# fernandezdaniel/MOBOCMF

Hardware: AMD Instinct MI355X
Metric: ELBO steps/sec (MFDGP d=8 M=512 N=8192 S=8) (higher is better)
Workload: dtype f64

## Files before the change

### include/mobocmf_hip.h

```cpp
#ifndef MOBOCMF_HIP_H
#define MOBOCMF_HIP_H

#include <stddef.h>
#include <stdint.h>

#ifdef __cplusplus
extern "C" {
#endif

typedef void* mobocmf_stream_t;

#define MOBOCMF_MAX_D 32
#define MOBOCMF_MAX_XDIV 48

enum {
    MOBOCMF_OK = 0,
    MOBOCMF_BAD_ARG = 1,
    MOBOCMF_WORKSPACE_TOO_SMALL = 2,
    MOBOCMF_HIP_ERROR = 3,
    MOBOCMF_NOT_PD = 4,
    MOBOCMF_BAD_ARCH = 5
};

typedef struct mobocmf_tuning {
    uint32_t struct_size;
    int32_t small_gemm_max;
    int32_t small_panel_max;
    int32_t tile_rows;
    int32_t pair_mode;
    int32_t mid_gemm_max;
    int32_t mid_gemm_waves;
    int32_t syrk_workgroups;
    int32_t sparse_backward;
    int32_t potrf_cols;
} mobocmf_tuning;
int mobocmf_tuning_init(mobocmf_tuning* t);

typedef struct {
    int32_t kind;
    int32_t d;
    int32_t M;
    int32_t xdiv;
    int64_t Np;
    int32_t branch;
    int32_t want_dx;
    double jitter;
    double min_var;
    int32_t phase;
    int32_t reserved;
    const mobocmf_tuning* tuning;
    void* const* probe_events;
} mobocmf_layer_desc;
#define MOBOCMF_PROBE_EVENTS 11

#define MOBOCMF_PHASE_ALL 0
#define MOBOCMF_PHASE_CHAIN 1
#define MOBOCMF_PHASE_PANEL 2
#define MOBOCMF_PHASE_CHAIN_ONLY 3
#define MOBOCMF_PHASE_PANEL_INPUTS 4

int mobocmf_version(void);
int mobocmf_device_arch_ok(void);

int mobocmf_layer_workspace_bytes(const mobocmf_layer_desc* desc, size_t* saved_bytes, size_t* scratch_bytes);

int mobocmf_layer_chain_state_bytes(const mobocmf_layer_desc* desc, size_t* bytes);

// ... 381 lines not shown
```

### mobocmf_amd/_lib.py

```python
import ctypes
import os

_HERE = os.path.dirname(os.path.abspath(__file__))
LIB_PATH = os.environ.get("MOBOCMF_HIP_LIB") or os.path.join(_HERE, "csrc", "libmobocmf_hip.so")

OK, BAD_ARG, WORKSPACE_TOO_SMALL, HIP_ERROR, NOT_PD, BAD_ARCH = range(6)
_ERR = {1: "MOBOCMF_BAD_ARG", 2: "MOBOCMF_WORKSPACE_TOO_SMALL", 3: "MOBOCMF_HIP_ERROR", 4: "MOBOCMF_NOT_PD",
        5: "MOBOCMF_BAD_ARCH"}


class Tuning(ctypes.Structure):
    _fields_ = [("struct_size", ctypes.c_uint32), ("small_gemm_max", ctypes.c_int32), ("small_panel_max", ctypes.c_int32),
                ("tile_rows", ctypes.c_int32), ("pair_mode", ctypes.c_int32), ("mid_gemm_max", ctypes.c_int32),
                ("mid_gemm_waves", ctypes.c_int32), ("syrk_workgroups", ctypes.c_int32), ("sparse_backward", ctypes.c_int32),
                ("potrf_cols", ctypes.c_int32)]
    KNOBS = tuple(n for n, _ in _fields_[1:])

    def copy(self):
        t = Tuning()
        ctypes.memmove(ctypes.byref(t), ctypes.byref(self), ctypes.sizeof(Tuning))
        return t


PROBE_EVENTS = 11


class LayerDesc(ctypes.Structure):
    _fields_ = [("kind", ctypes.c_int32), ("d", ctypes.c_int32), ("M", ctypes.c_int32), ("xdiv", ctypes.c_int32),
                ("Np", ctypes.c_int64), ("branch", ctypes.c_int32), ("want_dx", ctypes.c_int32),
                ("jitter", ctypes.c_double), ("min_var", ctypes.c_double), ("phase", ctypes.c_int32),
                ("reserved", ctypes.c_int32), ("tuning", ctypes.POINTER(Tuning)), ("probe_events", ctypes.c_void_p)]


TINY_MAX_LAYERS, TINY_MAX_M, TINY_MAX_D = 3, 32, 8
COOP_MAX_M = 128
FROZEN_MAX_M = 512
FROZEN_SPLIT_MAX_M = 1024
STEP_GRADIENTS, STEP_UPDATE, STEP_FORWARD, STEP_INPUT_GRADIENTS, STEP_COUPLED = range(5)
STEP_CHAIN_VALID = 16


class TinyModel(ctypes.Structure):
    _L = TINY_MAX_LAYERS
    _fields_ = [("L", ctypes.c_int32), ("M", ctypes.c_int32), ("d", ctypes.c_int32), ("S", ctypes.c_int32),
                ("N", ctypes.c_int32), ("rows", ctypes.c_int32 * _L), ("trainable", ctypes.c_uint32 * _L),
                ("branch", ctypes.c_int32),
                ("x", ctypes.c_void_p), ("y", ctypes.c_void_p), ("fid", ctypes.c_void_p), ("Zx", ctypes.c_void_p),
                ("raw", (ctypes.c_void_p * 7) * _L), ("m", ctypes.c_void_p * _L), ("L_S", ctypes.c_void_p * _L),
                ("raw_noise", ctypes.c_void_p * _L), ("noise_lo", ctypes.c_double * _L), ("noise_hi", ctypes.c_double * _L),
# ... 215 lines not shown
```

### mobocmf_amd/csrc/api.hip

```cpp
#include "common.h"

static const mobocmf_tuning kDefaultTuning = {(uint32_t)sizeof(mobocmf_tuning), 384, 512, 0, 0, 1024, 32, 0, 1, 0};
static thread_local const mobocmf_tuning* t_tuning = nullptr;
static thread_local void* const* t_probe = nullptr;
const mobocmf_tuning& tune() { return t_tuning ? *t_tuning : kDefaultTuning; }
bool tuning_ok(const mobocmf_tuning* t) {
    if (!t) return true;
    return t->struct_size == sizeof(mobocmf_tuning) && t->small_gemm_max >= 1 && t->small_gemm_max <= 512 &&
           t->small_panel_max >= 1 && t->small_panel_max <= 512 && (t->tile_rows == 0 || t->tile_rows == 64 || t->tile_rows == 128) &&
           t->pair_mode >= 0 && t->pair_mode <= 2 && t->mid_gemm_max >= 0 && t->mid_gemm_max <= 4096 &&
           (t->mid_gemm_waves == 4 || t->mid_gemm_waves == 8 || t->mid_gemm_waves == 32) &&
           (t->syrk_workgroups == 0 || (t->syrk_workgroups >= 16 && t->syrk_workgroups <= 4096)) &&
           (t->sparse_backward == 0 || t->sparse_backward == 1) && (t->potrf_cols == 0 || t->potrf_cols == 1 || t->potrf_cols == 4);
}
TuneScope::TuneScope(const mobocmf_tuning* t, void* const* probe) : prev_t(t_tuning), prev_p(t_probe) {
    t_tuning = t;
    t_probe = probe;
}
TuneScope::~TuneScope() {
    t_tuning = prev_t;
    t_probe = prev_p;
}
void probe_at(int i, hipStream_t s) {
    if (t_probe && i < MOBOCMF_PROBE_EVENTS && t_probe[i]) (void)hipEventRecord((hipEvent_t)t_probe[i], s);
}
static void set_pairing(GemmArgs& g) { g.pair_mode = tune().pair_mode; }
static int panel_tile_rows(int, int64_t) { return tune().tile_rows; }

#define TRY(x)              \
    do {                    \
        int _rc = (x);      \
        if (_rc) return _rc; \
    } while (0)

namespace {

struct Bump {
    uintptr_t base;
    size_t off, cap;
    bool ok;
    Bump(void* p, size_t c) : base((uintptr_t)p), off(0), cap(c), ok(true) {}
    double* take(int64_t n) {
        size_t bytes = ((size_t)n * sizeof(double) + 255) & ~(size_t)255;
        if (bytes > cap || off > cap - bytes) { ok = false; off += bytes; return nullptr; }
        double* r = base ? (double*)(base + off) : nullptr;
        off += bytes;
        return r;
    }
};

struct Dims {
    int M, Mp, nrb, H;
    int64_t N, Np, nbase;
    int splitk;
    dim3 ggrid_mn, ggrid_mm;
};

GemmArgs gemm_args(const double* A, int64_t lda, const double* B, int64_t ldb, double* C, int64_t ldc, int Mr, int64_t Nc,
                   int64_t Kd, int tri, double alpha) {
    GemmArgs g = {};
    g.A = A; g.lda = lda; g.B = B; g.ldb = ldb; g.C = C; g.ldc = ldc;
    g.Mr = Mr; g.Nc = Nc; g.Kd = Kd; g.tri = tri; g.alpha = alpha;
    return g;
}

int syrk_splitk(int Mp, int64_t Np, int* sD) {
    const int nrb = Mp / TILE;
    const int64_t nF = (int64_t)nrb * (nrb - 1) / 2, nD = nrb, ksteps = Np / 16;
    int cap = (int)(ksteps / 8);
    if (cap > 128) cap = 128;
    if (cap < 1) cap = 1;
    *sD = 0;
    if (nF == 0) {
        int sk = 512 < cap ? 512 : cap;
        if (sk >= 8) sk &= ~7;
        return sk;
    }
    int budget = tune().syrk_workgroups;
    if (budget <= 0) budget = Np <= 16384 ? 256 : 512;
    double best = 1e30;
    int bF = 1, bD = 1;
    for (int f = 1; f <= cap; ++f)
        for (int d = 1; d <= f; ++d) {
            if (nF * f + nD * d > budget) break;
            const double cf = (double)((ksteps + f - 1) / f), cd = 0.625 * (double)((ksteps + d - 1) / d);
            double c = cf > cd ? cf : cd;
            if ((f & 7) || (d & 7)) c *= 1.10;
            c += 1e-3 * (f + d);
            if (c < best) { best = c; bF = f; bD = d; }
        }
    *sD = bD;
    return bF;
}
int64_t syrk_slab_elems(int Mp, int64_t Np) {
    int sD;
    const int sk = syrk_splitk(Mp, Np, &sD);
    return (int64_t)(sk > 16 ? sk : 16) * Mp * Mp;
}
int weighted_syrk(const double* A, int64_t lda, const double* w, int Mp, int64_t Np, double* slabs, double* H,
                  const int32_t* skip, const double* fallback, const int32_t* kact, hipStream_t s) {
    const int64_t mm = (int64_t)Mp * Mp;
    GemmArgs ga = gemm_args(A, lda, A, lda, slabs, Mp, Mp, Mp, Np, TRI_NONE, 1.0);
    ga.bscale = w; ga.lower_out = 1; ga.sym_out = 1; ga.slab_stride = mm; ga.skip_if_zero = skip;
    ga.kact = kact;
    int sD = 0;
    const int sF = syrk_splitk(Mp, Np, &sD);
    const int nsl = gemm_nt_slabs(ga, sF);
    if (gemm_nt_is_small(ga) && !skip) {
        ga.C = H; ga.ldc = Mp; ga.sym_full = 1;
        return launch_gemm(ga, true, 1, s);
    }
    if (nsl > 1) ga.splitk_diag = sD;
    TRY(launch_gemm(ga, true, nsl, s));
    return launch_reduce_slabs_sym(slabs, mm, nsl, (nsl > 1 && sD > 0) ? sD : nsl, H, Mp, skip, fallback, s);
}

int weighted_syrk_pair(const double* A, int64_t lda, const double* w, const double* w2, int Mp, int64_t Np, double* slabs,
                       double* slabs2, double* H, double* Hc, const int32_t* flag, const int32_t* kact, hipStream_t s) {
    const int64_t mm = (int64_t)Mp * Mp;
    GemmArgs ga = gemm_args(A, lda, A, lda, slabs, Mp, Mp, Mp, Np, TRI_NONE, 1.0);
    ga.bscale = w; ga.lower_out = 1; ga.sym_out = 1; ga.slab_stride = mm;
    int sD = 0;
    const int sF = syrk_splitk(Mp, Np, &sD);
    const int nsl = gemm_nt_slabs(ga, sF);
    if (gemm_nt_is_small(ga)) {
        ga.C = H; ga.ldc = Mp; ga.sym_full = 1;
        ga.bscale2 = w2; ga.C2 = Hc;
        return launch_gemm(ga, true, 1, s);
    }
    if (nsl <= 1) {
        TRY(weighted_syrk(A, lda, w, Mp, Np, slabs, H, nullptr, nullptr, kact, s));
        return weighted_syrk(A, lda, w2, Mp, Np, slabs, Hc, flag, H, kact, s);
    }
    ga.splitk_diag = sD;
    ga.dual_flag = flag; ga.bscale2 = w2; ga.C2 = slabs2; ga.kact = kact;
    TRY(launch_gemm(ga, true, nsl, s));
    return launch_reduce_slabs_sym2(slabs, slabs2, mm, nsl, sD > 0 ? sD : nsl, H, Hc, Mp, flag, s);
}

bool valid_desc(const mobocmf_layer_desc* d) {
    return d && tuning_ok(d->tuning) && (d->kind == 0 || d->kind == 1) && d->d >= 1 && d->d <= MOBOCMF_MAX_D && d->M >= 1 && d->xdiv >= 1 &&
           d->xdiv <= MOBOCMF_MAX_XDIV && d->Np >= 1 && d->Np % d->xdiv == 0 && (d->branch == 0 || d->branch == 1) && d->phase >= 0 &&
           d->phase <= MOBOCMF_PHASE_PANEL_INPUTS;
}

Dims dims_of(const mobocmf_layer_desc* d) {
    Dims D;
    D.M = d->M;
    D.Mp = (int)round_up(d->M, TILE);
    D.nrb = D.Mp / TILE;
    D.N = d->Np;
    D.Np = round_up(d->Np, TILE);
    D.nbase = d->Np / d->xdiv;
    D.H = hyp_len(d->kind, d->d);
    { int sD; D.splitk = syrk_splitk(D.Mp, D.Np, &sD); }
    GramArgs g = {};
// ... 997 lines not shown
```

### mobocmf_amd/csrc/gemm_f64.hip

```cpp
#include "common.h"
#include <type_traits>
#include <atomic>

typedef double v4f64 __attribute__((ext_vector_type(4)));
typedef double v2f64 __attribute__((ext_vector_type(2)));

#define BM 128
#define BN 128
#define BK 16
#define KL_MAX 1024
#define TILE_ELEMS (BM * BK)

#define IMG_SWZ(row) ((((row) >> 1) & 1) | ((((row) >> 3) & 1) << 2))


template <int CTRL>
__device__ __forceinline__ double dpp_mov(double v) {
    int lo = __double2loint(v), hi = __double2hiint(v);
    lo = __builtin_amdgcn_update_dpp(0, lo, CTRL, 0xF, 0xF, false);
    hi = __builtin_amdgcn_update_dpp(0, hi, CTRL, 0xF, 0xF, false);
    return __hiloint2double(hi, lo);
}
__device__ __forceinline__ double row16_sum(double v) {
    v += dpp_mov<0xB1>(v);
// ... 27 lines not shown
__device__ unsigned long long* g_stamp_buf = nullptr;
extern "C" int mobocmf_debug_set_stamps(unsigned long long* p) {
    return hipMemcpyToSymbol(HIP_SYMBOL(g_stamp_buf), &p, sizeof(p)) == hipSuccess ? 0 : 3;
}
#define STAMP(i)                                                                                            \
    do {                                                                                                    \
        if (g_stamp_buf && threadIdx.x == 0) g_stamp_buf[(int64_t)blockIdx.x * 32 + (i)] = __builtin_amdgcn_s_memrealtime(); \
    } while (0)
#define STAMP_ID()                                                                                          \
    do {                                                                                                    \
        if (g_stamp_buf && threadIdx.x == 0) {                                                              \
            unsigned hw, xcc;                                                                               \
            asm volatile("s_getreg_b32 %0, hwreg(HW_REG_HW_ID)" : "=s"(hw));                               \
            asm volatile("s_getreg_b32 %0, hwreg(HW_REG_XCC_ID)" : "=s"(xcc));                             \
            g_stamp_buf[(int64_t)blockIdx.x * 32 + 15] = ((unsigned long long)xcc << 32) | hw;              \
        }                                                                                                   \
    } while (0)
#define STEP_STAMPS_DECL unsigned long long sst[10] = {0, 0, 0, 0, 0, 0, 0, 0, 0, 0};
#define STEP_STAMP(i) do { if (sbase >= 0) sst[sbase + (i)] = __builtin_amdgcn_s_memrealtime(); } while (0)
#define STEP_STAMPS_FLUSH                                                                                   \
    do {                                                                                                    \
        if (g_stamp_buf && threadIdx.x == 0)                                                                \
            for (int q = 0; q < 10; ++q) g_stamp_buf[(int64_t)blockIdx.x * 32 + 16 + q] = sst[q];           \
    } while (0)
#else
#define STAMP(i)
#define STAMP_ID()
#define STEP_STAMPS_DECL
#define STEP_STAMP(i)
#define STEP_STAMPS_FLUSH
#endif

template <bool B_T, bool TRI, int EPI, int RM>
__global__ __launch_bounds__(256, RM == 64 ? 3 : 2) void gemm_f64_kernel(GemmArgs g, int nrb, int64_t ncb, int splitk, int pair) {
    static_assert(RM == 128 || (RM == 64 && !B_T), "tile heights: 128, or 64 for the A B form");
    constexpr int MT = RM / 32;
    constexpr int A_ELEMS = RM * BK;
    constexpr int STAGE_ELEMS = A_ELEMS + TILE_ELEMS;
    __shared__ __attribute__((aligned(16))) double lds[2 * STAGE_ELEMS];
    __shared__ int kl[B_T ? KL_MAX : 1];
    __shared__ int kl_wsum[4];
    if (g.skip_if_zero && *g.skip_if_zero == 0) return;
    STAMP(0);
    STAMP_ID();
    int64_t id = blockIdx.x;
    if (g.dual_flag) {
        const int64_t half = (int64_t)(gridDim.x >> 1);
        if (id >= half) {
            if (*g.dual_flag == 0) return;
            id -= half;
            g.bscale = g.bscale2;
            g.C = g.C2;
        }
    }
    int rb, z = 0, sk_eff = splitk;
    int64_t cb;
    if (g.batched) {
        z = blockIdx.z;
        cb = id / nrb;
        rb = nrb - 1 - (int)(id % nrb);
    } else if (splitk > 1 && g.lower_out && g.splitk_diag > 0) {
        const int64_t nF = (int64_t)nrb * (nrb - 1) / 2, nblkF = nF * splitk;
        const bool diag = id >= nblkF;
        const int64_t id2 = diag ? id - nblkF : id, nT = diag ? nrb : nF;
        sk_eff = diag ? g.splitk_diag : splitk;
        int64_t t;
        if ((sk_eff & 7) == 0 && (nblkF & 7) == 0) {
            const int64_t xcd = id2 & 7, seq = id2 >> 3;
            t = seq % nT;
            z = (int)((seq / nT) * 8 + xcd);
        } else {
            t = id2 % nT;
            z = (int)(id2 / nT);
        }
        if (diag) {
            rb = (int)t;
            cb = t;
        } else {
            int r = 1;
            while ((int64_t)r * (r + 1) / 2 <= t) ++r;
            rb = r;
            cb = t - (int64_t)r * (r - 1) / 2;
        }
    } else if (splitk > 1) {
        const int64_t ntile = g.lower_out ? (int64_t)nrb * (nrb + 1) / 2 : (int64_t)nrb * ncb;
        int64_t t;
        if ((splitk & 7) == 0) {
            const int64_t xcd = id & 7, seq = id >> 3;
            t = seq % ntile;
            z = (int)((seq / ntile) * 8 + xcd);
        } else {
            t = id % ntile;
            z = (int)(id / ntile);
        }
        if (g.lower_out) {
            int r = 0;
            while ((int64_t)(r + 1) * (r + 2) / 2 <= t) ++r;
            rb = r;
            cb = t - (int64_t)r * (r + 1) / 2;
        } else {
            cb = t / nrb;
            rb = (int)(t % nrb);
        }
    } else {
        const int nslot = pair ? (nrb + 1) / 2 : nrb;
        int sl;
        if ((ncb & 7) == 0) {
            int64_t xcd = id & 7, slot = id >> 3;
            cb = (slot / nslot) * 8 + xcd;
            sl = (int)(slot % nslot);
        } else {
            cb = id / nslot;
            sl = (int)(id % nslot);
        }
        rb = pair ? sl : nrb - 1 - sl;
    }
    if (g.lower_out && cb > rb) return;

    const double* A = g.A;
    const double* B = g.B;
    double* C = g.C;
    if (g.batched) {
        const int zl = g.zlayers > 1 ? z % g.zlayers : 0;
        const int zb = g.zlayers > 1 ? z / g.zlayers : z;
        A += zb * g.strideA + zl * g.zsA;
        B += zb * g.strideB + zl * g.zsB;
        C += zb * g.strideC + zl * g.zsC;
    }
    if (!g.batched && splitk > 1) {
        C += z * g.slab_stride;
        if (g.zlayers > 1) {
            A += blockIdx.z * g.zsA;
            B += blockIdx.z * g.zsB;
            C += blockIdx.z * g.zsC;
        }
    }
    const int nparts = (pair && rb != nrb - 1 - rb) ? 2 : 1;
    const int rb_first = rb;

    const int tid = threadIdx.x;
    const int lane = tid & 63;
    const int wave = __builtin_amdgcn_readfirstlane(tid >> 6);
    const int wr = wave >> 1, wc = wave & 1;
    const int li = lane & 15, lk = lane >> 4;

    if constexpr (!B_T) {
        if (g.colact && g.colact[cb] == 0) {
            if (EPI == EPI_DA && g.rowdot_part) {
                for (int part = 0; part < nparts; ++part) {
                    const int rbp = part == 0 ? rb_first : nrb - 1 - rb_first;
                    for (int i = tid; i < 2 * RM; i += 256)
                        g.rowdot_part[((int64_t)cb * 2 + i / RM) * g.Mr + (int64_t)rbp * RM + i % RM] = 0.0;
                }
            }
            return;
        }
    }

    const int a_row = tid >> 3;
    const int a_lchk = (tid & 7) ^ IMG_SWZ(a_row);
    const double* Ag0 = A + (int64_t)a_row * g.lda + a_lchk * 2;
    const double* Bg = B_T ? B + (cb * BN + a_row) * g.ldb + a_lchk * 2
                           : B + (int64_t)wave * g.ldb + cb * BN;
    auto stage = [&](const double* Ag, int64_t k, int buf) {
        double* As = lds + buf * STAGE_ELEMS;
        double* Bs = As + A_ELEMS;
#pragma unroll
        for (int r = 0; r < RM / 32; ++r) glds16(Ag + (int64_t)(32 * r) * g.lda + k, As + (r * 4 + wave) * 128);
        if (B_T) {
#pragma unroll
            for (int r = 0; r < 4; ++r) glds16(Bg + (int64_t)(32 * r) * g.ldb + k, Bs + (r * 4 + wave) * 128);
        } else {
#pragma unroll
            for (int r = 0; r < 4; ++r)
                glds16(Bg + (k + 4 * r) * g.ldb + lane * 2, Bs + (r * 4 + wave) * 128);
        }
    };

    const int swA = IMG_SWZ(li);
    const int colP0 = ((2 * lk + 0) ^ swA) << 1, colP1 = ((2 * lk + 1) ^ swA) << 1;
    const int a_base = (wr * 16 + li) * BK;
    const int bt_base = (wc * 16 + li) * BK;
    const int bn_base = (4 * lk) * BN + wc * 64 + 2 * li;

  STEP_STAMPS_DECL
  for (int part = 0; part < nparts; ++part) {
    const bool upper = (g.tri & TRI_UPPER_A) != 0;
    const bool long_first_is_high = !upper;
    rb = ((part == 0) == long_first_is_high) ? nrb - 1 - rb_first : rb_first;
    if (nparts == 1) rb = rb_first;
    const bool rev = TRI && nparts == 2 && (upper ? part == 0 : part == 1);
    int64_t k0 = 0, k1 = g.Kd;
    if (g.tri & TRI_LOWER_A) {
        int64_t e = (int64_t)(rb + 1) * RM;
        if (k1 > e) k1 = e;
    }
    if (g.tri & TRI_UPPER_A) {
        int64_t b = (int64_t)rb * RM;
        if (k0 < b) k0 = b;
    }
    if (g.tri & TRI_LOWER_B) {
// ... 21 lines not shown
                    const int v = __shfl_up(inc, off);
                    if (lane >= off) inc += v;
                }
                if (lane == 63) kl_wsum[wave] = inc;
                __syncthreads();
                int ord = inc - cnt;
                for (int w = 0; w < wave; ++w) ord += kl_wsum[w];
                const int64_t nkt = (int64_t)(kl_wsum[0] + kl_wsum[1] + kl_wsum[2] + kl_wsum[3]) * (128 / BK);
                const int64_t per = (nkt + sk_eff - 1) / sk_eff;
                const int64_t tb = z * per < nkt ? z * per : nkt, te = tb + per < nkt ? tb + per : nkt;
                ct0 = tb;
                co0 = (int)(tb / (128 / BK));
                const int co1 = te > tb ? (int)((te - 1) / (128 / BK)) : co0 - 1;
                for (int b = rb0; b < rb1; ++b)
                    if (g.kact[b] != 0) {
                        if (ord >= co0 && ord <= co1 && ord - co0 < KL_MAX) kl[ord - co0] = b;
                        ++ord;
                    }
                __syncthreads();
                compact = true;
                sliced = true;
                k0 = 0;
                k1 = (te - tb) * BK;
            }
        }
        if (!sliced) {
            int64_t nkt = k1 > k0 ? (k1 - k0) / BK : 0;
            int64_t per = (nkt + sk_eff - 1) / sk_eff;
            int64_t b = k0 + z * per * BK, e = b + per * BK;
            k0 = b < k1 ? b : k1;
            k1 = e < k1 ? e : k1;
        }
    }
    const double* Ag = Ag0 + (int64_t)rb * RM * g.lda;

    v4f64 acc[MT][4];
#pragma unroll
    for (int i = 0; i < MT; ++i)
#pragma unroll
        for (int j = 0; j < 4; ++j) acc[i][j] = (v4f64){0.0, 0.0, 0.0, 0.0};

    const int64_t nk = (k1 > k0) ? (k1 - k0) / BK : 0;
#define KSTEP(KT) (rev ? nk - 1 - (KT) : (KT))
    auto koff = [&](int64_t kt) -> int64_t {
        if (B_T && compact) {
            const int64_t t = ct0 + kt;
            return (int64_t)kl[(int)(t / (128 / BK)) - co0] * 128 + (t % (128 / BK)) * BK;
        }
        return k0 + KSTEP(kt) * BK;
    };
#define KOFF(KT) koff(KT)
    if (nk > 0) stage(Ag, KOFF(0), 0);

    asm volatile("s_waitcnt vmcnt(0)" ::: "memory");
    __syncthreads();
    STAMP(1 + 4 * part);
    v4f64 w_nxt = (v4f64){1.0, 1.0, 1.0, 1.0};
    if (B_T && g.bscale && nk > 0) w_nxt = *(const v4f64*)(g.bscale + KOFF(0) + 4 * lk);
    v2f64 fa[MT][2];
    double fb[4][4];
#define LOAD_A16(MT_)                                                                                       \
    fa[MT_][0] = *(const v2f64*)(As + a_base + (MT_) * 32 * BK + colP0);                                    \
    fa[MT_][1] = *(const v2f64*)(As + a_base + (MT_) * 32 * BK + colP1);
#define LOAD_B16                                                                                            \
    if (B_T) {                                                                                              \
        _Pragma("unroll") for (int t = 0; t < 4; ++t) {                                                    \
            const v2f64 v0 = *(const v2f64*)(Bs + bt_base + t * 32 * BK + colP0);                           \
// ... 34 lines not shown
        LOAD_B16                                                                                            \
        LOAD_A16(0)                                                                                         \
        STAGE_NEXT                                                                                          \
        LOAD_A16(MT - 1)                                                                                    \
        if constexpr (MT == 4) {                                                                            \
            LOAD_A16(1)                                                                                     \
            LOAD_A16(2)                                                                                     \
        }                                                                                                   \
        __builtin_amdgcn_sched_barrier(0);                                                                  \
        MMA(0)                                                                                              \
        if constexpr (MT == 4) {                                                                            \
            MMA(1)                                                                                          \
            MMA(2)                                                                                          \
        }                                                                                                   \
        MMA(MT - 1)                                                                                         \
                                                                             \
        __builtin_amdgcn_sched_barrier(0);
#define KSTEP_LE                                                                                            \
        LOAD_B16                                                                                            \
        LOAD_A16(0)                                                                                         \
        STAGE_NEXT                                                                                          \
        LOAD_A16(1) LOAD_A16(2) LOAD_A16(3)                                                                 \
        __builtin_amdgcn_sched_barrier(0);                                                                  \
        MMA16(0, 1) MMA16(1, 2) MMA16(2, 3) MMA16(3, 4)                                                     \
        __builtin_amdgcn_sched_barrier(0);
#define KSTEP_LT                                                                                            \
        LOAD_B16                                                                                            \
        LOAD_A16(1)                                                                                         \
        STAGE_NEXT                                                                                          \
        LOAD_A16(2) LOAD_A16(3)                                                                             \
        __builtin_amdgcn_sched_barrier(0);                                                                  \
        MMA16(1, 1) MMA16(2, 2) MMA16(3, 3)                                                                 \
        __builtin_amdgcn_sched_barrier(0);
#define STAGE_LOOP(KT0, KT1, COND, BODY)                                                                    \
    for (int64_t kt = (KT0); kt < (KT1); ++kt) {                                                            \
        const int buf = (int)(kt & 1);                                                                      \
        const v4f64 w4 = w_nxt;                \
        const int sbase = (part == 0 && kt == nk - 2) ? 0 : (part == 0 && kt == 4) ? 5 : -1;                \
        (void)sbase;                                                                                        \
        STEP_STAMP(0);                                                                                      \
        const double* As = lds + buf * STAGE_ELEMS;                                                         \
        const double* Bs = As + A_ELEMS;                                                                    \
        int act = 15;                                                                                       \
        if ((COND) == 1) {                                                                                  \
            const int64_t kk = k0 + KSTEP(kt) * BK;                                                         \
            const int64_t r0 = (int64_t)rb * RM + wr * 16;                                                  \
            act = 0;                                                                                        \
            _Pragma("unroll") for (int mt = 0; mt < MT; ++mt) {                                            \
                const bool nz = (g.tri & TRI_LOWER_A) ? (kk <= r0 + mt * 32 + 15) : (kk + 15 >= r0 + mt * 32); \
                act |= nz ? (1 << mt) : 0;                                                                  \
            }                                                                                               \
            act = __builtin_amdgcn_readfirstlane(act);                                                      \
        }                                                                                                   \
        (void)act;                                                                                          \
        BODY                                                                                                \
        STEP_STAMP(2);                                                                                      \
            \
        asm volatile("s_waitcnt vmcnt(0) lgkmcnt(0)" ::: "memory");                                         \
        STEP_STAMP(3);                                                                                      \
        __syncthreads();                                                                                    \
        STEP_STAMP(4);                                                                                      \
    }
    if (TRI) {
        const int64_t nd = nk < RM / BK ? nk : RM / BK;
        const bool diag_first = upper != rev;
        const int64_t d0 = ((g.tri & (TRI_LOWER_A | TRI_UPPER_A)) && diag_first) ? nd : 0;
        const int64_t d1 = ((g.tri & (TRI_LOWER_A | TRI_UPPER_A)) && !diag_first) ? nk - nd : nk;
        STAGE_LOOP(0, d0, 1, KSTEP_STD(MMA_IF))
        STAMP(2 + 4 * part);
        STAGE_LOOP(d0, d1, 0, KSTEP_STD(MMA_ALL))
        STAMP(3 + 4 * part);
        STAGE_LOOP(d1, nk, 1, KSTEP_STD(MMA_IF))
    } else {
        bool done = false;
        if constexpr (B_T) {
            if (g.sym_out && g.lower_out && rb == cb) {
                const int wave_u = __builtin_amdgcn_readfirstlane(wave);
                if (wave_u == 1) {
                    STAGE_LOOP(0, nk, 0, KSTEP_LT)
                } else {
                    STAGE_LOOP(0, nk, 0, KSTEP_LE)
                }
                done = true;
            }
        }
        if (!done) { STAGE_LOOP(0, nk, 0, KSTEP_STD(MMA_ALL)) }
    }
#undef STAGE_LOOP
#undef KSTEP
#undef KOFF
#undef KSTEP_STD
#undef STAGE_NEXT
#undef KSTEP_LE
#undef KSTEP_LT
#undef MMA_IF
#undef MMA_ALL
#undef LOAD_A16
#undef LOAD_B16
#undef MMA16

    STAMP(4 + 4 * part);

    const int64_t row0 = (int64_t)rb * RM + wr * 16 + lk;
    const int64_t col0 = cb * BN + (B_T ? wc * 16 + li : wc * 64 + 2 * li);
    const int ccol = B_T ? wc * 16 + li : wc * 64 + 2 * li;
#define COLOFF(nt) (B_T ? (nt) * 32 : ((nt) >> 1) * 32 + ((nt) & 1))
    if (EPI == EPI_DA && !B_T) {
        v2f64 gm[2], cg[2], cs[2];
#pragma unroll
        for (int h = 0; h < 2; ++h) {
            gm[h] = *(const v2f64*)(g.gmu + col0 + 32 * h);
            cg[h] = *(const v2f64*)(g.cgv + col0 + 32 * h);
            cs[h] = (v2f64){1.0, 1.0};
        }
        if (g.bscale) {
#pragma unroll
            for (int h = 0; h < 2; ++h) cs[h] = *(const v2f64*)(g.bscale + col0 + 32 * h);
        }
        double rdkeep = 0.0;
#pragma unroll
        for (int mt = 0; mt < MT; ++mt) {
            v2f64 av[2][4];
            double ar[4];
#pragma unroll
            for (int r = 0; r < 4; ++r) {
                ar[r] = g.avec[row0 + mt * 32 + 4 * r];
#pragma unroll
                for (int h = 0; h < 2; ++h)
                    av[h][r] = *(const v2f64*)(g.Aaux + (row0 + mt * 32 + 4 * r) * g.ldc + col0 + 32 * h);
            }
#pragma unroll
            for (int r = 0; r < 4; ++r) {
                double rd = 0.0;
#pragma unroll
                for (int h = 0; h < 2; ++h) {
                    const v2f64 a = av[h][r];
// ... 37 lines not shown
                for (int r = 0; r < 4; ++r) {
                    const double v = g.alpha * acc[mt][nt][r];
                    sq[nt] += v * v;
                    dt[nt] += ar[mt][r] * v;
                }
        if (part == 0) STAMP(11);
#pragma unroll
        for (int nt = 0; nt < 4; ++nt) {
            sq[nt] = rows4_sum(sq[nt]);
            if (want_dot) dt[nt] = rows4_sum(dt[nt]);
        }
        if (lk == 0) {
            const int64_t prow = ((int64_t)rb * 2 + wr) * g.Nc + col0;
            if (B_T) {
#pragma unroll
                for (int nt = 0; nt < 4; ++nt) {
                    g.colsq_part[prow + COLOFF(nt)] = sq[nt];
                    if (want_dot) g.coldot_part[prow + COLOFF(nt)] = dt[nt];
                }
            } else {
#pragma unroll
                for (int h = 0; h < 2; ++h) {
                    *(v2f64*)(g.colsq_part + prow + 32 * h) = (v2f64){sq[2 * h], sq[2 * h + 1]};
                    if (want_dot) *(v2f64*)(g.coldot_part + prow + 32 * h) = (v2f64){dt[2 * h], dt[2 * h + 1]};
                }
            }
        }
        if (part == 0) STAMP(12);
        __builtin_amdgcn_sched_barrier(0);
    }
#define STORE_TILE(ST, ST2, ACCUM)                                                                          \
    {                                                                                                       \
        double* cp = C + row0 * g.ldc + col0;                                                               \
        const int64_t step4 = 4 * g.ldc, step_mt = 32 * g.ldc - 16 * g.ldc;                                 \
        _Pragma("unroll") for (int mt = 0; mt < MT; ++mt) {                                                \
            _Pragma("unroll") for (int r = 0; r < 4; ++r) {                                                \
                if (B_T) {                                                                                  \
                    _Pragma("unroll") for (int nt = 0; nt < 4; ++nt) {                                     \
                        double v = g.alpha * acc[mt][nt][r];                                                \
                        if (ACCUM) v += cp[COLOFF(nt)];                                                     \
                        ST(v, cp + COLOFF(nt));                                                             \
                    }                                                                                       \
                } else {                                                                                    \
                    _Pragma("unroll") for (int h = 0; h < 2; ++h) {                                        \
                        v2f64 v;                                                                            \
                        v[0] = g.alpha * acc[mt][2 * h][r];                                                 \
                        v[1] = g.alpha * acc[mt][2 * h + 1][r];                                             \
                        if (ACCUM) v += *(const v2f64*)(cp + 32 * h);                                       \
                        ST2(v, (v2f64*)(cp + 32 * h));                                                      \
                    }                                                                                       \
                }                                                                                           \
                cp += step4;                                                                                \
            }                                                                                               \
            cp += step_mt;                                                                                  \
        }                                                                                                   \
    }
#define ST_PLAIN(v, p) (*(p) = (v))
#define ST_STREAM(v, p) __builtin_nontemporal_store((v), (p))
    if (g.accumulate) { STORE_TILE(ST_PLAIN, ST_PLAIN, 1) }
    else if (g.stream_out) { STORE_TILE(ST_STREAM, ST_STREAM, 0) }
    else { STORE_TILE(ST_PLAIN, ST_PLAIN, 0) }
#undef STORE_TILE
    if (part == 0) STAMP(13);

#undef COLOFF
    STAMP(9 + part);
  }
  STEP_STAMPS_FLUSH;
}

static bool small_panel_ok(const GemmArgs& g, bool B_T, int splitk);
template <int EPI> static int launch_small_panel(const GemmArgs& g, hipStream_t s);
static bool small_gemm_ok(const GemmArgs& g, bool B_T);
static int launch_small_gemm(const GemmArgs& g, bool B_T, hipStream_t s);

static int tile_rows(const GemmArgs& g, bool B_T, int splitk) {
    if (B_T || splitk > 1 || g.batched || g.lower_out || g.zlayers > 1) return BM;
    if (g.rm == 64 || g.rm == BM) return g.rm;
    if (!(g.tri & (TRI_LOWER_A | TRI_UPPER_A))) return BM;
    const int64_t pairs128 = (int64_t)((g.Mr / BM + 1) / 2) * (g.Nc / BN);
    return pairs128 >= 512 ? BM : 64;
}

int launch_gemm(const GemmArgs& g0, bool B_T, int splitk, hipStream_t s) {
    GemmArgs g = g0;
    if (g.Mr % BM || g.Nc % 16 || g.Kd % BK) return MOBOCMF_BAD_ARG;
    if (B_T || g.batched || splitk > 1) g.colact = nullptr;
    if (g.kact) {
        const int sk_min = (g.lower_out && g.splitk_diag > 0 && g.splitk_diag < splitk) ? g.splitk_diag : splitk;
        const int64_t nb = g.Kd / 128;
        if (!B_T || g.batched || splitk <= 1 || g.zlayers > 1 || g.Kd % 128 || (g.tri & (TRI_LOWER_B | TRI_UPPER_B)) ||
            (nb + sk_min - 1) / sk_min + 2 > KL_MAX)
            g.kact = nullptr;
    }
    if (!B_T && ((g.ldc & 1) || ((uintptr_t)g.C & 15))) return MOBOCMF_BAD_ARG;
    if (small_panel_ok(g, B_T, splitk)) {
        if (g.epi == EPI_COLSTATS) return launch_small_panel<EPI_COLSTATS>(g, s);
        if (g.epi == EPI_DA) return launch_small_panel<EPI_DA>(g, s);
        return launch_small_panel<EPI_STORE>(g, s);
    }
    if (g.Nc % BN) return MOBOCMF_BAD_ARG;
    if (B_T && splitk <= 1 && small_gemm_ok(g, true)) return launch_small_gemm(g, true, s);
    if (!B_T && g.batched > 1 && splitk <= 1 && small_gemm_ok(g, false)) return launch_small_gemm(g, false, s);
    const int rm = tile_rows(g, B_T, splitk);
    int nrb = g.Mr / rm;
    int64_t ncb = g.Nc / BN;
    dim3 grid;
    int pair = 0;
    if (g.batched) {
        grid = dim3((unsigned)(nrb * ncb), 1, (unsigned)(g.batched * (g.zlayers > 1 ? g.zlayers : 1)));
        splitk = 1;
    } else if (splitk > 1) {
        int64_t ntile = g.lower_out ? (int64_t)nrb * (nrb + 1) / 2 : (int64_t)nrb * ncb;
        if (g.lower_out && g.splitk_diag > 0) ntile = 0;
        const int64_t nblk = ntile ? ntile * splitk : (int64_t)nrb * (nrb - 1) / 2 * splitk + (int64_t)nrb * g.splitk_diag;
        grid = dim3((unsigned)(g.dual_flag ? 2 * nblk : nblk), 1, (unsigned)(g.zlayers > 1 ? g.zlayers : 1));
    } else {
        const bool can_pair = (g.tri & (TRI_LOWER_A | TRI_UPPER_A)) && !g.lower_out && nrb > 1;
        if (rm == 64) pair = (can_pair && (int64_t)(nrb / 2) * ncb >= 256) ? 1 : 0;
        else pair = (can_pair && (int64_t)nrb * ncb > 512) ? 1 : 0;
        if (g.pair_mode == 1) pair = 0;
        if (g.pair_mode == 2 && (g.tri & (TRI_LOWER_A | TRI_UPPER_A)) && !g.lower_out && nrb > 1) pair = 1;
        grid = dim3((unsigned)((pair ? (nrb + 1) / 2 : nrb) * ncb), 1, 1);
        splitk = 1;
    }
    const bool tri = (g.tri & (TRI_LOWER_A | TRI_UPPER_A)) != 0 || g.epi == EPI_STORE;
#define LAUNCH(BT, TR, EP, RM_) hipLaunchKernelGGL((gemm_f64_kernel<BT, TR, EP, RM_>), grid, dim3(256), 0, s, g, nrb, ncb, splitk, pair)
    if (B_T) {
        if (g.epi != EPI_STORE) return MOBOCMF_BAD_ARG;
        LAUNCH(true, false, EPI_STORE, 128);
    } else if (rm == 64) {
        if (g.epi == EPI_COLSTATS) LAUNCH(false, true, EPI_COLSTATS, 64);
        else if (g.epi == EPI_DA) LAUNCH(false, true, EPI_DA, 64);
        else LAUNCH(false, true, EPI_STORE, 64);
    } else if (tri) {
        if (g.epi == EPI_COLSTATS) LAUNCH(false, true, EPI_COLSTATS, 128);
        else if (g.epi == EPI_DA) LAUNCH(false, true, EPI_DA, 128);
        else LAUNCH(false, true, EPI_STORE, 128);
    } else {
        if (g.epi == EPI_COLSTATS) LAUNCH(false, false, EPI_COLSTATS, 128);
        else if (g.epi == EPI_DA) LAUNCH(false, false, EPI_DA, 128);
        else LAUNCH(false, false, EPI_STORE, 128);
    }
#undef LAUNCH
    return hipGetLastError() == hipSuccess ? MOBOCMF_OK : MOBOCMF_HIP_ERROR;
}

int gemm_colstat_rows(const GemmArgs& g) {
    if (small_panel_ok(g, false, 1)) return 2 * (g.Mr / BM);
    return 2 * (g.Mr / tile_rows(g, false, 1));
}

__global__ void reduce_slabs_kernel(const double* slabs, int64_t slab_stride, int nslab, double* out, int64_t ld,
                                    int rows, int64_t cols, double scale, int lower_only, int tril, int accumulate,
                                    int64_t zs_slabs, int64_t zs_out) {
    int64_t idx = (int64_t)blockIdx.x * blockDim.x + threadIdx.x;
    if (idx >= (int64_t)rows * cols) return;
    slabs += blockIdx.z * zs_slabs;
    out += blockIdx.z * zs_out;
    int i = (int)(idx / cols);
    int64_t j = idx % cols;
    if (lower_only && (j / TILE) > (i / TILE)) {
        if (tril && !accumulate) out[(int64_t)i * ld + j] = 0.0;
// ... 710 lines not shown
```

### mobocmf_amd/functional.py

```python
import contextlib
import ctypes
import os
import threading

import torch

from . import _lib
from ._lib import LayerDesc

JITTER = 1e-6
MIN_VARIANCE = 1e-10

_scratch = {}


def _stream():
    return ctypes.c_void_p(torch.cuda.current_stream().cuda_stream)


def _ptr(t):
    return ctypes.c_void_p(0 if t is None else t.data_ptr())


def _prep(t):
# ... 58 lines not shown
        del _scratch[key]
    for key in [k for k in _side_streams if k[1] == stream.cuda_stream]:
        del _side_streams[key]


def hyp_len(kind, d):
    return 1 + d if kind == 0 else 5 + 2 * d


PHASE_ALL, PHASE_CHAIN, PHASE_PANEL, PHASE_CHAIN_ONLY, PHASE_PANEL_INPUTS = 0, 1, 2, 3, 4


_TUNING_DEFAULT = None
_tuning_tls = threading.local()


def _default_tuning():
    global _TUNING_DEFAULT
    if _TUNING_DEFAULT is None:
        t = _lib.Tuning()
        _lib.check(_lib.load().mobocmf_tuning_init(ctypes.byref(t)), "mobocmf_tuning_init")
        _TUNING_DEFAULT = t
    return _TUNING_DEFAULT


def current_tuning():
    t = getattr(_tuning_tls, "override", None)
    return (t if t is not None else _default_tuning()).copy()


def _set_default(**kw):
    t = _default_tuning()
    for k, v in kw.items():
        assert k in _lib.Tuning.KNOBS, k
        setattr(t, k, int(v))


@contextlib.contextmanager
def tuning(**kw):
    prev = getattr(_tuning_tls, "override", None)
    t = current_tuning()
    for k, v in kw.items():
        if k not in _lib.Tuning.KNOBS:
            raise TypeError("unknown tuning knob %r" % k)
        setattr(t, k, int(v))
    _tuning_tls.override = t
    try:
        yield t
    finally:
        _tuning_tls.override = prev


_probe_tls = threading.local()


@contextlib.contextmanager
def probe_events(table, layer=None):
    prev = getattr(_probe_tls, "cur", None)
    _probe_tls.cur = (table, layer)
    try:
        yield
    finally:
        _probe_tls.cur = prev


def _probe_for(layer):
    cur = getattr(_probe_tls, "cur", None)
    if cur is None or (cur[1] is not None and layer is not None and cur[1] != layer):
        return None
    return cur[0]


def make_desc(kind, d, M, Np, xdiv=1, branch=0, want_dx=False, jitter=JITTER, min_var=MIN_VARIANCE, phase=PHASE_ALL,
              tune=None, probe=None):
    if not 1 <= d <= _lib.MAX_D:
        raise _lib.MobocmfError("mobocmf_amd: a layer takes 1..%d input dimensions (got %d): the Gram kernels keep one "
# ... 1278 lines not shown

def raise_if_abandoned(pivot, what="Cholesky"):
    if pivot < 0:
        raise InLaunchWaitAbandoned("%s: the one-launch form abandoned a bounded in-launch wait (its workgroups were not resident "
                                    "together); repeat the call with F.tuning(potrf_cols=4) or less concurrent work" % what)


def gemm_colstat_rows(Mr, Nc, Kd, tri=0, tune=None):
    rows = ctypes.c_int32()
    snap = tune if tune is not None else current_tuning()
    _lib.check(_lib.load().mobocmf_gemm_colstat_rows(tri, Mr, Nc, Kd, ctypes.byref(snap), ctypes.byref(rows)),
               "mobocmf_gemm_colstat_rows")
    return rows.value


def set_mid_gemm_max(n=1024):
    if not 0 <= int(n) <= 4096:
        raise _lib.MobocmfError("set_mid_gemm_max: 0..4096")
    _set_default(mid_gemm_max=n)


def set_mid_gemm_waves(n=32):
    if int(n) not in (4, 8, 32):
        raise _lib.MobocmfError("set_mid_gemm_waves: 4 | 8 | 32")
    _set_default(mid_gemm_waves=n)


def set_syrk_workgroups(n=0):
    if int(n) != 0 and not 16 <= int(n) <= 4096:
        raise _lib.MobocmfError("set_syrk_workgroups: 0 | 16..4096")
    _set_default(syrk_workgroups=n)


def set_sparse_backward(on=True):
    _set_default(sparse_backward=1 if on else 0)


_block_act_tls = threading.local()


def set_block_activity(act=None):
    if act is not None:
        assert act.dtype == torch.int32 and act.is_cuda and act.is_contiguous()
    _block_act_tls.act = act


def set_tile_rows(rows=0, pair_mode=0):
    if int(rows) not in (0, 64, 128) or not 0 <= int(pair_mode) <= 2:
        raise _lib.MobocmfError("set_tile_rows: rows 0 | 64 | 128, pair_mode 0..2")
    _set_default(tile_rows=rows, pair_mode=pair_mode)


def set_potrf_cols(cols=0):
    if int(cols) not in (0, 1, 4):
        raise _lib.MobocmfError("set_potrf_cols: 0 | 1 | 4")
    _set_default(potrf_cols=cols)


def set_tuning(small_gemm_max=0, small_panel_max=0):
    if int(small_gemm_max) > 512 or int(small_panel_max) > 512:
        raise _lib.MobocmfError("set_tuning: the small kernels serve dimensions <= 512")
    if small_gemm_max > 0:
        _set_default(small_gemm_max=small_gemm_max)
    if small_panel_max > 0:
        _set_default(small_panel_max=small_panel_max)

# ... 541 lines not shown
```

Measured before the change: 1069.

## Add 64-row tiles for the k-sliced weighted SYRK to halve diagonal waste

Adds a 64-row A·B^T tile variant of the GEMM kernel for the split-k symmetric weighted SYRK. Off-diagonal 128-wide column blocks are split into two 64-row halves, and each diagonal block is split into two half-tiles that only compute the lower-triangle MMAs, using per-wave roles. The variant is picked by default when Np <= 32768, and a second split-k search rebalances slice counts for the doubled tile count. The aim is less redundant upper-triangle work and better occupancy. The cost is more workgroups and smaller tiles, which lowers arithmetic intensity.

```diff
diff --git a/include/mobocmf_hip.h b/include/mobocmf_hip.h
--- a/include/mobocmf_hip.h
+++ b/include/mobocmf_hip.h
@@ -33,6 +33,7 @@
     int32_t syrk_workgroups;
     int32_t sparse_backward;
     int32_t potrf_cols;
+    int32_t syrk_tile_rows;
 } mobocmf_tuning;
 int mobocmf_tuning_init(mobocmf_tuning* t);
 
diff --git a/mobocmf_amd/_lib.py b/mobocmf_amd/_lib.py
--- a/mobocmf_amd/_lib.py
+++ b/mobocmf_amd/_lib.py
@@ -13,8 +13,10 @@
     _fields_ = [("struct_size", ctypes.c_uint32), ("small_gemm_max", ctypes.c_int32), ("small_panel_max", ctypes.c_int32),
                 ("tile_rows", ctypes.c_int32), ("pair_mode", ctypes.c_int32), ("mid_gemm_max", ctypes.c_int32),
                 ("mid_gemm_waves", ctypes.c_int32), ("syrk_workgroups", ctypes.c_int32), ("sparse_backward", ctypes.c_int32),
-                ("potrf_cols", ctypes.c_int32)]
-    KNOBS = tuple(n for n, _ in _fields_[1:])
+                ("potrf_cols", ctypes.c_int32), ("syrk_tile_rows", ctypes.c_int32)]
+    KNOBS = tuple(n for n, _ in _fields_[1:10])
+    KNOBS_APPENDED = tuple(n for n, _ in _fields_[10:])
+    ALL_KNOBS = KNOBS + KNOBS_APPENDED
 
     def copy(self):
         t = Tuning()
diff --git a/mobocmf_amd/csrc/api.hip b/mobocmf_amd/csrc/api.hip
--- a/mobocmf_amd/csrc/api.hip
+++ b/mobocmf_amd/csrc/api.hip
@@ -1,6 +1,6 @@
 #include "common.h"
 
-static const mobocmf_tuning kDefaultTuning = {(uint32_t)sizeof(mobocmf_tuning), 384, 512, 0, 0, 1024, 32, 0, 1, 0};
+static const mobocmf_tuning kDefaultTuning = {(uint32_t)sizeof(mobocmf_tuning), 384, 512, 0, 0, 1024, 32, 0, 1, 0, 0};
 static thread_local const mobocmf_tuning* t_tuning = nullptr;
 static thread_local void* const* t_probe = nullptr;
 const mobocmf_tuning& tune() { return t_tuning ? *t_tuning : kDefaultTuning; }
@@ -11,7 +11,8 @@
            t->pair_mode >= 0 && t->pair_mode <= 2 && t->mid_gemm_max >= 0 && t->mid_gemm_max <= 4096 &&
            (t->mid_gemm_waves == 4 || t->mid_gemm_waves == 8 || t->mid_gemm_waves == 32) &&
            (t->syrk_workgroups == 0 || (t->syrk_workgroups >= 16 && t->syrk_workgroups <= 4096)) &&
-           (t->sparse_backward == 0 || t->sparse_backward == 1) && (t->potrf_cols == 0 || t->potrf_cols == 1 || t->potrf_cols == 4);
+           (t->sparse_backward == 0 || t->sparse_backward == 1) && (t->potrf_cols == 0 || t->potrf_cols == 1 || t->potrf_cols == 4) &&
+           (t->syrk_tile_rows == 0 || t->syrk_tile_rows == 64 || t->syrk_tile_rows == 128);
 }
 TuneScope::TuneScope(const mobocmf_tuning* t, void* const* probe) : prev_t(t_tuning), prev_p(t_probe) {
     t_tuning = t;
@@ -64,31 +65,43 @@
     return g;
 }
 
-int syrk_splitk(int Mp, int64_t Np, int* sD) {
+static int syrk_tile_rows(int Mp, int64_t Np) {
+    const int t = tune().syrk_tile_rows;
+    if (t == 64 || t == TILE) return t;
+    (void)Mp;
+    return Np <= 32768 ? 64 : TILE;
+}
+static void syrk_slices(int64_t nF, int64_t nD, int64_t ksteps, int cap, int budget, double share, int* bF, int* bD) {
+    double best = 1e30;
+    *bF = 1; *bD = 1;
+    for (int f = 1; f <= cap; ++f)
+        for (int d = 1; d <= f; ++d) {
+            if (nF * f + nD * d > budget) break;
+            const double cf = (double)((ksteps + f - 1) / f), cd = share * (double)((ksteps + d - 1) / d);
+            double c = cf > cd ? cf : cd;
+            if ((f & 7) || (d & 7)) c *= 1.10;
+            c += 1e-3 * (f + d);
+            if (c < best) { best = c; *bF = f; *bD = d; }
+        }
+}
+int syrk_splitk(int Mp, int64_t Np, int* sD, int* rm_out = nullptr) {
     const int nrb = Mp / TILE;
     const int64_t nF = (int64_t)nrb * (nrb - 1) / 2, nD = nrb, ksteps = Np / 16;
     int cap = (int)(ksteps / 8);
     if (cap > 128) cap = 128;
     if (cap < 1) cap = 1;
+    const int rm = syrk_tile_rows(Mp, Np);
+    if (rm_out) *rm_out = rm;
     *sD = 0;
     if (nF == 0) {
         int sk = 512 < cap ? 512 : cap;
         if (sk >= 8) sk &= ~7;
         return sk;
     }
-    int budget = tune().syrk_workgroups;
-    if (budget <= 0) budget = Np <= 16384 ? 256 : 512;
-    double best = 1e30;
+    const int forced = tune().syrk_workgroups;
     int bF = 1, bD = 1;
-    for (int f = 1; f <= cap; ++f)
-        for (int d = 1; d <= f; ++d) {
-            if (nF * f + nD * d > budget) break;
-            const double cf = (double)((ksteps + f - 1) / f), cd = 0.625 * (double)((ksteps + d - 1) / d);
-            double c = cf > cd ? cf : cd;
-            if ((f & 7) || (d & 7)) c *= 1.10;
-            c += 1e-3 * (f + d);
-            if (c < best) { best = c; bF = f; bD = d; }
-        }
+    syrk_slices(nF, nD, ksteps, cap, forced > 0 ? forced : (Np <= 16384 ? 256 : 512), 0.625, &bF, &bD);
+    if (rm == 64) syrk_slices(2 * nF, 2 * nD, ksteps, bF, forced > 0 ? forced : 512, 0.625, &bF, &bD);
     *sD = bD;
     return bF;
 }
@@ -104,7 +117,7 @@
     ga.bscale = w; ga.lower_out = 1; ga.sym_out = 1; ga.slab_stride = mm; ga.skip_if_zero = skip;
     ga.kact = kact;
     int sD = 0;
-    const int sF = syrk_splitk(Mp, Np, &sD);
+    const int sF = syrk_splitk(Mp, Np, &sD, &ga.rm);
     const int nsl = gemm_nt_slabs(ga, sF);
     if (gemm_nt_is_small(ga) && !skip) {
         ga.C = H; ga.ldc = Mp; ga.sym_full = 1;
@@ -121,7 +134,7 @@
     GemmArgs ga = gemm_args(A, lda, A, lda, slabs, Mp, Mp, Mp, Np, TRI_NONE, 1.0);
     ga.bscale = w; ga.lower_out = 1; ga.sym_out = 1; ga.slab_stride = mm;
     int sD = 0;
-    const int sF = syrk_splitk(Mp, Np, &sD);
+    const int sF = syrk_splitk(Mp, Np, &sD, &ga.rm);
     const int nsl = gemm_nt_slabs(ga, sF);
     if (gemm_nt_is_small(ga)) {
         ga.C = H; ga.ldc = Mp; ga.sym_full = 1;
diff --git a/mobocmf_amd/csrc/gemm_f64.hip b/mobocmf_amd/csrc/gemm_f64.hip
--- a/mobocmf_amd/csrc/gemm_f64.hip
+++ b/mobocmf_amd/csrc/gemm_f64.hip
@@ -83,8 +83,9 @@
 #endif
 
 template <bool B_T, bool TRI, int EPI, int RM>
-__global__ __launch_bounds__(256, RM == 64 ? 3 : 2) void gemm_f64_kernel(GemmArgs g, int nrb, int64_t ncb, int splitk, int pair) {
-    static_assert(RM == 128 || (RM == 64 && !B_T), "tile heights: 128, or 64 for the A B form");
+__global__ __launch_bounds__(256, (RM == 64 && !B_T) ? 3 : 2) void gemm_f64_kernel(GemmArgs g, int nrb, int64_t ncb, int splitk, int pair) {
+    static_assert(RM == 128 || RM == 64, "tile heights: 128 or 64");
+    static_assert(!(RM == 64 && B_T) || (!TRI && EPI == EPI_STORE), "64-row A B^T tiles: the k-sliced symmetric product only");
     constexpr int MT = RM / 32;
     constexpr int A_ELEMS = RM * BK;
     constexpr int STAGE_ELEMS = A_ELEMS + TILE_ELEMS;
@@ -106,7 +107,38 @@
     }
     int rb, z = 0, sk_eff = splitk;
     int64_t cb;
-    if (g.batched) {
+    int64_t a_row_base = -1;
+    int a_row_r1 = 32;
+    if constexpr (RM == 64 && B_T) {
+        const int n128 = nrb >> 1;
+        const int64_t nF = (int64_t)n128 * (n128 - 1), nblkF = nF * splitk;
+        const bool diag = id >= nblkF;
+        const int64_t id2 = diag ? id - nblkF : id, nT = diag ? nrb : nF;
+        sk_eff = diag ? g.splitk_diag : splitk;
+        int64_t t;
+        if ((sk_eff & 7) == 0 && (nblkF & 7) == 0) {
+            const int64_t xcd = id2 & 7, seq = id2 >> 3;
+            t = seq % nT;
+            z = (int)((seq / nT) * 8 + xcd);
+        } else {
+            t = id2 % nT;
+            z = (int)(id2 / nT);
+        }
+        if (z >= sk_eff) return;
+        if (diag) {
+            const int h = (int)(t & 1);
+            rb = (int)t;
+            cb = t >> 1;
+            a_row_base = cb * BN + 32 * h;
+            a_row_r1 = 96 - 64 * h;
+        } else {
+            const int64_t p = t >> 1;
+            int r = 1;
+            while ((int64_t)r * (r + 1) / 2 <= p) ++r;
+            rb = 2 * r + (int)(t & 1);
+            cb = p - (int64_t)r * (r - 1) / 2;
+        }
+    } else if (g.batched) {
         z = blockIdx.z;
         cb = id / nrb;
         rb = nrb - 1 - (int)(id % nrb);
@@ -166,7 +198,7 @@
         }
         rb = pair ? sl : nrb - 1 - sl;
     }
-    if (g.lower_out && cb > rb) return;
+    if (g.lower_out && cb * BN > (int64_t)rb * RM) return;
 
     const double* A = g.A;
     const double* B = g.B;
@@ -217,7 +249,8 @@
         double* As = lds + buf * STAGE_ELEMS;
         double* Bs = As + A_ELEMS;
 #pragma unroll
-        for (int r = 0; r < RM / 32; ++r) glds16(Ag + (int64_t)(32 * r) * g.lda + k, As + (r * 4 + wave) * 128);
+        for (int r = 0; r < RM / 32; ++r)
+            glds16(Ag + (int64_t)((RM == 64 && B_T ? a_row_r1 : 32) * r) * g.lda + k, As + (r * 4 + wave) * 128);
         if (B_T) {
 #pragma unroll
             for (int r = 0; r < 4; ++r) glds16(Bg + (int64_t)(32 * r) * g.ldb + k, Bs + (r * 4 + wave) * 128);
@@ -305,7 +338,7 @@
             k1 = e < k1 ? e : k1;
         }
     }
-    const double* Ag = Ag0 + (int64_t)rb * RM * g.lda;
+    const double* Ag = Ag0 + (a_row_base >= 0 ? a_row_base : (int64_t)rb * RM) * g.lda;
 
     v4f64 acc[MT][4];
 #pragma unroll
@@ -406,6 +439,14 @@
         __builtin_amdgcn_sched_barrier(0);                                                                  \
         MMA16(1, 1) MMA16(2, 2) MMA16(3, 3)                                                                 \
         __builtin_amdgcn_sched_barrier(0);
+#define KSTEP_SYM64(J0, J1)                                                                                 \
+        LOAD_B16                                                                                            \
+        LOAD_A16(0)                                                                                         \
+        STAGE_NEXT                                                                                          \
+        LOAD_A16(1)                                                                                         \
+        __builtin_amdgcn_sched_barrier(0);                                                                  \
+        MMA16(0, J0) MMA16(1, J1)                                                                           \
+        __builtin_amdgcn_sched_barrier(0);
 #define STAGE_LOOP(KT0, KT1, COND, BODY)                                                                    \
     for (int64_t kt = (KT0); kt < (KT1); ++kt) {                                                            \
         const int buf = (int)(kt & 1);                                                                      \
@@ -447,7 +488,21 @@
         STAGE_LOOP(d1, nk, 1, KSTEP_STD(MMA_IF))
     } else {
         bool done = false;
-        if constexpr (B_T) {
+        if constexpr (B_T && RM == 64) {
+            if (a_row_base >= 0) {
+                const int role = __builtin_amdgcn_readfirstlane(((rb & 1) << 1) | (wave == 1 ? 1 : 0));
+                if (role == 0) {
+                    STAGE_LOOP(0, nk, 0, KSTEP_SYM64(1, 4))
+                } else if (role == 1) {
+                    STAGE_LOOP(0, nk, 0, KSTEP_SYM64(0, 3))
+                } else if (role == 2) {
+                    STAGE_LOOP(0, nk, 0, KSTEP_SYM64(2, 3))
+                } else {
+                    STAGE_LOOP(0, nk, 0, KSTEP_SYM64(1, 2))
+                }
+                done = true;
+            }
+        } else if constexpr (B_T) {
             if (g.sym_out && g.lower_out && rb == cb) {
                 const int wave_u = __builtin_amdgcn_readfirstlane(wave);
                 if (wave_u == 1) {
@@ -467,6 +522,7 @@
 #undef STAGE_NEXT
 #undef KSTEP_LE
 #undef KSTEP_LT
+#undef KSTEP_SYM64
 #undef MMA_IF
 #undef MMA_ALL
 #undef LOAD_A16
@@ -475,7 +531,7 @@
 
     STAMP(4 + 4 * part);
 
-    const int64_t row0 = (int64_t)rb * RM + wr * 16 + lk;
+    const int64_t row0 = (a_row_base >= 0 ? a_row_base : (int64_t)rb * RM) + wr * 16 + lk;
     const int64_t col0 = cb * BN + (B_T ? wc * 16 + li : wc * 64 + 2 * li);
     const int ccol = B_T ? wc * 16 + li : wc * 64 + 2 * li;
 #define COLOFF(nt) (B_T ? (nt) * 32 : ((nt) >> 1) * 32 + ((nt) & 1))
@@ -579,7 +635,7 @@
 #define STORE_TILE(ST, ST2, ACCUM)                                                                          \
     {                                                                                                       \
         double* cp = C + row0 * g.ldc + col0;                                                               \
-        const int64_t step4 = 4 * g.ldc, step_mt = 32 * g.ldc - 16 * g.ldc;                                 \
+        const int64_t step4 = 4 * g.ldc, step_mt = ((RM == 64 && B_T ? a_row_r1 : 32) - 16) * g.ldc;        \
         _Pragma("unroll") for (int mt = 0; mt < MT; ++mt) {                                                \
             _Pragma("unroll") for (int r = 0; r < 4; ++r) {                                                \
                 if (B_T) {                                                                                  \
@@ -622,7 +678,8 @@
 static int launch_small_gemm(const GemmArgs& g, bool B_T, hipStream_t s);
 
 static int tile_rows(const GemmArgs& g, bool B_T, int splitk) {
-    if (B_T || splitk > 1 || g.batched || g.lower_out || g.zlayers > 1) return BM;
+    if (B_T) return (g.rm == 64 && splitk > 1 && g.sym_out && g.lower_out && !g.batched && g.zlayers <= 1 && g.epi == EPI_STORE) ? 64 : BM;
+    if (splitk > 1 || g.batched || g.lower_out || g.zlayers > 1) return BM;
     if (g.rm == 64 || g.rm == BM) return g.rm;
     if (!(g.tri & (TRI_LOWER_A | TRI_UPPER_A))) return BM;
     const int64_t pairs128 = (int64_t)((g.Mr / BM + 1) / 2) * (g.Nc / BN);
@@ -657,6 +714,10 @@
     if (g.batched) {
         grid = dim3((unsigned)(nrb * ncb), 1, (unsigned)(g.batched * (g.zlayers > 1 ? g.zlayers : 1)));
         splitk = 1;
+    } else if (splitk > 1 && B_T && rm == 64) {
+        if (g.splitk_diag <= 0 || g.splitk_diag > splitk) g.splitk_diag = splitk;
+        const int64_t n128 = nrb / 2, nblk = n128 * (n128 - 1) * splitk + (int64_t)nrb * g.splitk_diag;
+        grid = dim3((unsigned)(g.dual_flag ? 2 * nblk : nblk), 1, 1);
     } else if (splitk > 1) {
         int64_t ntile = g.lower_out ? (int64_t)nrb * (nrb + 1) / 2 : (int64_t)nrb * ncb;
         if (g.lower_out && g.splitk_diag > 0) ntile = 0;
@@ -675,7 +736,8 @@
 #define LAUNCH(BT, TR, EP, RM_) hipLaunchKernelGGL((gemm_f64_kernel<BT, TR, EP, RM_>), grid, dim3(256), 0, s, g, nrb, ncb, splitk, pair)
     if (B_T) {
         if (g.epi != EPI_STORE) return MOBOCMF_BAD_ARG;
-        LAUNCH(true, false, EPI_STORE, 128);
+        if (rm == 64) LAUNCH(true, false, EPI_STORE, 64);
+        else LAUNCH(true, false, EPI_STORE, 128);
     } else if (rm == 64) {
         if (g.epi == EPI_COLSTATS) LAUNCH(false, true, EPI_COLSTATS, 64);
         else if (g.epi == EPI_DA) LAUNCH(false, true, EPI_DA, 64);
diff --git a/mobocmf_amd/functional.py b/mobocmf_amd/functional.py
--- a/mobocmf_amd/functional.py
+++ b/mobocmf_amd/functional.py
@@ -114,7 +114,7 @@
 def _set_default(**kw):
     t = _default_tuning()
     for k, v in kw.items():
-        assert k in _lib.Tuning.KNOBS, k
+        assert k in _lib.Tuning.ALL_KNOBS, k
         setattr(t, k, int(v))
 
 
@@ -123,7 +123,7 @@
     prev = getattr(_tuning_tls, "override", None)
     t = current_tuning()
     for k, v in kw.items():
-        if k not in _lib.Tuning.KNOBS:
+        if k not in _lib.Tuning.ALL_KNOBS:
             raise TypeError("unknown tuning knob %r" % k)
         setattr(t, k, int(v))
     _tuning_tls.override = t
@@ -1468,6 +1468,12 @@
     _set_default(syrk_workgroups=n)
 
 
+def set_syrk_tile_rows(rows=0):
+    if int(rows) not in (0, 64, 128):
+        raise _lib.MobocmfError("set_syrk_tile_rows: 0 | 64 | 128")
+    _set_default(syrk_tile_rows=rows)
+
+
 def set_sparse_backward(on=True):
     _set_default(sparse_backward=1 if on else 0)
 
```

Measured after the change: 1061. Within noise of the previous version (-0.7%).
